# mengyao/Complete-Striped-Smith-Waterman-Library

Hardware: AMD Instinct MI355X
Metric: GCUPS (higher is better)
Workload: dtype int16x2 in a column frame (value + phi(column); 32-bit adds on the packed pair, three-input maxima on the bit patterns); reference u8/int16 semantics; 1 GPU; BASELINE config 2: 100k x 150 bp reads vs 1 Mb target; 2/-2/3/1, score_size 2, flag 0; reads_per_gpu=100000, read_len=150, ref_len=1000000

## Files before the change

complete-striped-smith-waterman-library_amd/csrc/lanes.h:

```cpp
#ifndef SSW_LANES_H
#define SSW_LANES_H

#include <stdint.h>

typedef uint32_t u32;
typedef short s16x2 __attribute__((ext_vector_type(2)));
typedef unsigned short u16x2 __attribute__((ext_vector_type(2)));
typedef uint32_t u32x4 __attribute__((ext_vector_type(4)));
typedef uint32_t u32x2 __attribute__((ext_vector_type(2)));

#ifdef SSW_SIMT_EMU
#include "simt_emu.h"
#else
#include <hip/hip_runtime.h>
#define SSW_DEV __device__ __forceinline__
#define SSW_DEVM __device__ __forceinline__
#define SSW_HD __host__ __device__ inline
#define SSW_DYN_LDS(name) extern __shared__ __attribute__((aligned(16))) unsigned char name[]

SSW_DEV u32 xl_row_shr1_zero(u32 v) { return (u32)__builtin_amdgcn_mov_dpp((int)v, 0x111, 0xf, 0xf, true); }
SSW_DEV u32 xl_row_shr1_keep(u32 keep, u32 v) { return (u32)__builtin_amdgcn_update_dpp((int)keep, (int)v, 0x111, 0xf, 0xf, false); }
SSW_DEV u32 xl_row_shr1_umax(u32 v, u32 b)
{
	u32 r;
// ... 159 lines not shown
{
	const int l = emu::cur->lane, i = l & 15;
	int src = i;
	if (CTRL < 0x100) src = (i & ~3) | ((CTRL >> (2 * (i & 3))) & 3);
	else if ((CTRL & 0x1f0) == 0x100) src = i + (CTRL & 15);
	else if ((CTRL & 0x1f0) == 0x110) src = i - (CTRL & 15);
	else src = (i - (CTRL & 15)) & 15;
	const bool ok = src >= 0 && src < 16 && ((BANK >> (i >> 2)) & 1);
	return emu::exchange(v, (l & ~15) | (src & 15), ok, old);
}
#else
template <int CTRL, int BANK> SSW_DEV u32 xl_dpp_banks(u32 old, u32 v) { return (u32)__builtin_amdgcn_update_dpp((int)old, (int)v, CTRL, 0xf, BANK, false); }
#endif
#define DPP_QUAD_SWAP1 0xB1
#define DPP_QUAD_SWAP2 0x4E

#endif
```

complete-striped-smith-waterman-library_amd/csrc/ssw_host.c:

```c
#include <stdlib.h>
#include <stdio.h>
#include <string.h>
#include <pthread.h>
#include "ssw.h"
#include "ssw_gpu.h"
#ifdef SSW_GPU_TEST_HOOKS
#include "ssw_gpu_diag.h"
#endif
#include "ssw_dev.h"

_Static_assert(sizeof(struct ssw_out_rec) == sizeof(ssw_gpu_result), "device record layout must equal ssw_gpu_result");
_Static_assert(sizeof(struct ssw_best_rec) == sizeof(ssw_gpu_best) && sizeof(ssw_gpu_best) == 16, "device record layout must equal ssw_gpu_best");

struct _profile {
	const int8_t* read;
	const int8_t* mat;
	int32_t readLen;
	int32_t n;
	int8_t score_size;
};

typedef struct { void* p; size_t cap; } dbuf;

typedef struct {
// ... 10 lines not shown
	int overlap;
	int no_track;
	int no_seg_reduce;
	int window_int16;
	int trace_wave;
	int trace_no_lds;
	int trace_waves;
	int trace_unblocked;
	int trace_many;
	int trace_early;
	int trace_w1max, trace_w4max, trace_headroom;
	int pipe_any_count;
	int pipe_low_prio;
	int pipe_parts;
	int no_fill_half;
	int no_pipe;
	int no_lit_spec;
	int trace_no_cls80;
	int trace_diag;
	int serial_buckets;
	int no_dbx;
	int no_tail;
	int no_band;
	int call_trace;
	int db_tsub, dbx_slab;
} ssw_knobs;

#define SSW_TSTREAMS 6
#define SSW_PSTREAMS 7
#define DB_STREAMS 4
// ... 40 lines not shown
#define CALL_TRACE(what) do { if (c->kn.call_trace) fprintf(stderr, "[ssw_gpu call] %9.3f ms  %s\n", dbg_ms(), what); } while (0)

#ifdef SSW_GPU_TEST_HOOKS
static int env_int(const char* name, int dflt) { const char* e = getenv(name); return e && e[0] ? atoi(e) : dflt; }
#endif
static int env_is(const char* name, char ch) { const char* e = getenv(name); return e && e[0] == ch; }
static void knobs_load(ssw_knobs* k)
{
	memset(k, 0, sizeof *k);
	k->debug = getenv("SSW_GPU_DEBUG") != 0;
	k->call_trace = env_is("SSW_GPU_CALL_TRACE", '1');
	k->db_chain_best = 1;
	k->trace_wave = -1;
	k->trace_many = 4096;
	k->trace_w1max = 96; k->trace_w4max = 256; k->trace_headroom = 8;
#ifdef SSW_GPU_TEST_HOOKS
	{ const int v = env_int("SSW_GPU_FRAME_K", 0); k->frame_k = v >= 16 ? v : 0; }
	k->queue_mode = env_is("SSW_GPU_QUEUE", 'j') ? 1 : env_is("SSW_GPU_QUEUE", 's') ? 2 : 0;
	{ const int v = env_int("SSW_GPU_QUEUE_WAVES", 0); k->queue_waves = v > 0 ? v : 0; }
	k->db_plain = env_is("SSW_GPU_DB_FORM", '0');
	k->db_chain_best = !env_is("SSW_GPU_DB_CHAIN_BEST", '0');
	k->xlanes16 = env_int("SSW_GPU_XLANES", 0) == 16;
	{ const int v = env_int("SSW_GPU_XR", 0); k->xr = v >= 1 && v <= 16 ? v : 0; }
	{ const int v = env_int("SSW_GPU_XR_WINDOW", 0); k->xr_window = v >= 1 && v <= 16 ? v : 0; }
	k->fill_plain = env_is("SSW_GPU_FILL_FORM", '0') || env_is("SSW_GPU_FILL_F16", '0');
	k->no_db = env_is("SSW_GPU_NO_DB", '1');
	k->overlap = env_is("SSW_GPU_OVERLAP", '1');
	k->no_track = env_is("SSW_GPU_NO_TRACK", '1');
	k->no_seg_reduce = env_is("SSW_GPU_SEG_REDUCE", '0');
	k->window_int16 = getenv("SSW_GPU_WINDOW_INT16") != 0;
	k->trace_wave = getenv("SSW_GPU_TRACE_WAVE") ? env_is("SSW_GPU_TRACE_WAVE", '1') : -1;
	k->trace_no_lds = env_is("SSW_GPU_TRACE_LDS", '0');
	{ const int v = env_int("SSW_GPU_TRACE_WAVES", 0); k->trace_waves = v == 1 || v == 4 || v == 16 ? v : 0; }
	k->trace_unblocked = env_is("SSW_GPU_TRACE_BLOCKED", '0');
	k->trace_diag = env_is("SSW_GPU_TRACE_DIAG", '1');
	if (getenv("SSW_GPU_TRACE_MANY")) k->trace_many = env_int("SSW_GPU_TRACE_MANY", 4096);
	k->serial_buckets = env_is("SSW_GPU_SERIAL_BUCKETS", '1');
	k->no_dbx = env_is("SSW_GPU_NO_DBX", '1');
	k->no_band = env_is("SSW_GPU_NO_BAND", '1');
	k->trace_no_cls80 = env_is("SSW_GPU_TRACE_CLS80", '0');
	k->no_lit_spec = env_is("SSW_GPU_LIT_SPEC", '0');
	k->no_pipe = env_is("SSW_GPU_PIPE", '0');
	k->no_fill_half = env_is("SSW_GPU_FILL_HALF", '0');
	k->pipe_low_prio = env_is("SSW_GPU_PIPE_PRIO", 'l');
	k->pipe_any_count = env_is("SSW_GPU_PIPE_EVEN", '0');
	{ const int v = env_int("SSW_GPU_TRACE_W1MAX", 0); if (v >= 2 && v <= 254) k->trace_w1max = v; }
	{ const int v = env_int("SSW_GPU_TRACE_W4MAX", 0); if (v >= 2 && v <= 3070) k->trace_w4max = v; }
	{ const int v = env_int("SSW_GPU_TRACE_HEADROOM", 0); if (v >= 2 && v <= 64) k->trace_headroom = v; }
	{ const int v = env_int("SSW_GPU_PIPE_PARTS", 0); k->pipe_parts = v >= 2 && v <= 8 ? v : 0; }
	k->trace_early = env_int("SSW_GPU_TRACE_EARLY", 0);
	k->no_tail = env_is("SSW_GPU_NO_TAIL", '1');
	{ const int v = env_int("SSW_GPU_DB_TSUB", 0); k->db_tsub = v > 0 ? v : 0; }
	{ const int v = env_int("SSW_GPU_DBX_SLAB", 0); k->dbx_slab = v > 0 ? v : 0; }
#endif
}
#ifdef SSW_GPU_TEST_HOOKS
int ssw_gpu_has_test_hooks(void) { return 1; }
// ... 451 lines not shown
	if (key <= SSW_RMAX) { b->R = key; b->strips = 1; b->P16 = 16 * key; b->lanes = 16; b->use_x = 0; return; }
	b->P16 = P16; b->lanes = g->xlanes; b->use_x = 1;
	b->strips = (P16 + g->rows - 1) / g->rows;
	b->R = (P16 + b->lanes * b->strips - 1) / (b->lanes * b->strips);
	if (b->lanes == 64 && b->strips > 1 && g->xrmax > 4 && !g->no_tail) {
		const int32_t rem = P16 - (b->strips - 1) * 64 * g->xrmax, need = (rem + 63) / 64, tr = need <= 1 ? 1 : need <= 2 ? 2 : need <= 4 ? 4 : 0;
		if (rem > 0 && tr > 0 && g->xrmax * (b->strips - 1) + tr < b->R * b->strips) { b->R = g->xrmax; b->tailR = tr; }
	}
}

typedef struct {
	int active, dbl, seg;
	int pipe;
	int32_t tile, halo, ntiles;
	int64_t maxcols, chunk;
	size_t cm_bytes, sg_bytes, bnd_bytes, cand_bytes, q_ints, cs_ints;
	size_t cm_off, sg_off, bnd_off, cand_off, q_off, cs_off;
} bplan;
typedef struct { int32_t key, sub, q; } keyed;
typedef struct { int32_t key, need, q; } tpend;
static int tpend_cmp(const void* a, const void* b)
{
	const tpend* x = (const tpend*)a; const tpend* y = (const tpend*)b;
	if (x->key != y->key) return x->key < y->key ? -1 : 1;
	return x->q < y->q ? -1 : x->q > y->q;
}
static int keyed_cmp(const void* a, const void* b)
{
	const keyed* x = (const keyed*)a; const keyed* y = (const keyed*)b;
	if (x->key != y->key) return x->key < y->key ? -1 : 1;
// ... 1205 lines not shown
	ssw_shim_event_record(e1, c->stream);
	c->tm.fill_launches++;
	for (int32_t q = 0; q < nq; ++q) c->tm.fill_cells += (Q->h_off[q + 1] - Q->h_off[q]) * (int64_t)refLen;
	note_fill_kernel(c, c->tm.fill_cells, &bc->best_fill_cells, "k_literal (lane model of the SSE2 kernels)", 0.0, 0, 1);
	return 0;
}

static void plan_bucket(const ssw_gpu_ctx* c, const batch_call* bc, const target_plan* tp, const bucket* B, bplan* P)
{
	const int32_t refLen = tp->refLen;
	const int64_t stride = tp->stride;
	const int32_t Pq = B->P16, halo_full = halo_for(Pq, bc->maxmat, bc->prm->gapE);
	const int use_x = B->use_x;
	const int gran = use_x ? 1 : 16;
	int32_t tile, halo, ntiles;
	int64_t want = 1;
	int small_call = 0;
	if ((int64_t)halo_full * 8 * gran < refLen) {
		int64_t launch_pairs = use_x ? B->npairs : (int64_t)(c->cm_budget / (size_t)(8 * stride));
		if (launch_pairs < 1) launch_pairs = 1;
		if (launch_pairs > B->npairs) launch_pairs = B->npairs;
		want = (4 * 32768 + B->npairs - 1) / B->npairs;
		if (!use_x && launch_pairs * ((want + 15) / 16) < 6000) want = 16 * ((6000 + launch_pairs - 1) / launch_pairs);
		int64_t maxt = refLen / ((int64_t)halo_full * 8);
		if (want > maxt) want = maxt;
		want = (want + gran - 1) / gran * gran; if (want < gran) want = gran;
	}
	{
		int64_t slots = use_x ? (int64_t)c->dev_wave_slots : (int64_t)c->dev_cus * (c->device_share > 1 ? 96 : 32);
		if (c->device_share > 1) { slots /= c->device_share; if (slots < 256) slots = 256; }
// ... 13 lines not shown
		ntiles = (refLen + tile - 1) / tile; halo = (halo_full + 15) / 16 * 16;
		if (ntiles <= 1) { ntiles = 1; tile = (refLen + 15) / 16 * 16; halo = 0; }
	}
	const int64_t maxcols = (((int64_t)tile + halo < refLen ? (int64_t)tile + halo : refLen) + 31) / 16 * 16;
	int64_t per_pair = 8 * stride + (use_x ? 16 * maxcols * ntiles : 0);
	int64_t chunk = (int64_t)(c->cm_budget / (size_t)per_pair);
	const int dbl = !use_x && chunk < B->npairs && c->kn.overlap;
	const int pipe = !use_x && !dbl && chunk < B->npairs && !c->kn.no_pipe;
	int parts = dbl || pipe ? 2 : 1;
	if (pipe && c->kn.pipe_parts) parts = c->kn.pipe_parts;
	if (parts > 1) chunk = (int64_t)((c->cm_budget / (size_t)parts) / (size_t)per_pair);
	if (chunk < 1) chunk = 1;
	if (chunk > B->npairs) chunk = B->npairs;
	if (!use_x && chunk < B->npairs) {
		const int64_t bpp = (ntiles + 15) / 16;
		int64_t nl = (B->npairs + chunk - 1) / chunk;
		if (pipe && parts > 1 && !c->kn.pipe_any_count && nl % parts) nl += parts - nl % parts;
		int64_t even = (B->npairs + nl - 1) / nl;
		const int64_t ncu = c->dev_cus;
		const int64_t unit = (ncu / (bpp > ncu ? ncu : bpp) > 0 ? ncu / (bpp > ncu ? ncu : bpp) : 1) * (B->half ? 2 : 1);
		even = (even + unit - 1) / unit * unit;
		if (even <= chunk) chunk = even;
		else if (chunk >= unit) chunk = chunk / unit * unit;
		if (B->half && (chunk & 1) && chunk > 1) --chunk;
	}
	memset(P, 0, sizeof *P);
	P->active = 1;
	P->tile = tile; P->halo = halo; P->ntiles = ntiles; P->maxcols = maxcols; P->chunk = chunk; P->dbl = dbl; P->pipe = pipe && chunk < B->npairs ? parts : 0;
	P->seg = !dbl && !c->kn.no_seg_reduce ;
	P->cm_bytes = ALIGN16(4 * stride * chunk) * (P->pipe ? P->pipe : 1);
	P->sg_bytes = P->seg ? ALIGN16(4 * tp->seg_stride * chunk) * (P->pipe ? P->pipe : 1) : 0;
	P->bnd_bytes = use_x ? ALIGN16(16 * maxcols * ntiles * chunk) : 0;
	P->cand_bytes = use_x ? ALIGN16(32 * ntiles * chunk) : 0;
	if (use_x && B->lanes == 64) { P->q_ints = chainq_queue_ints(chunk * ntiles * B->strips); P->cs_ints = chainq_cands_ints(chunk * ntiles * B->strips); }
}

static void plan_target(const ssw_gpu_ctx* c, const batch_call* bc, target_plan* tp, int allow_conc)
{
	tp->max_chunk = 1; tp->nact = 0;
	tp->tot_cm = tp->tot_sg = tp->tot_bnd = tp->tot_cand = tp->tot_q = tp->tot_cs = 0;
	tp->max_cm = tp->max_sg = tp->max_bnd = tp->max_cand = 0;
// ... 86 lines not shown
	if (!half || B->use_x || fa->form != 3 || !ssw_frame_params(&c->kn, top, prm->gapO, prm->gapE, bc->minmat, 8, &hb, &hk)) return 0;
	fa->fr_base = hb; fa->fr_kmask = hk;
	return 1;
}

static void reduce_args_for(const ssw_gpu_ctx* c, const batch_call* bc, const target_plan* tp, const bucket* B, const bplan* P, int32_t p0, int32_t np,
                            const fill_bufs* fb, ssw_reduce_args* ra)
{
	const ssw_gpu_params* prm = bc->prm;
	ra->cm16 = fb->cm16; ra->cm8 = fb->cm8; ra->cm_stride = tp->stride; ra->refLen = tp->refLen; ra->pairs = bc->d_pairs + B->first_pair + p0; ra->npairs = np;
	ra->qoff = bc->Q->d_off; ra->maskLen = prm->maskLen; ra->bias = bc->bias; ra->score_size = prm->score_size;
	ra->flag = prm->flag; ra->filters = prm->filters; ra->res = bc->d_res; ra->cand = bucket_cand(c, tp, B, P); ra->tile = P->tile; ra->ntiles = P->ntiles;
	ra->sg16 = fb->sg16; ra->sg8 = fb->sg8; ra->seg_stride = tp->seg_stride;
}

static int fill_launch(ssw_gpu_ctx* c, batch_call* bc, const target_plan* tp, int b, int32_t p0, int32_t np, const fill_bufs* fb, void* st, int* ndefer)
{
	const bucket* B = &bc->bk[b]; const bplan* P = &tp->bp[b];
	const ssw_gpu_params* prm = bc->prm;
	const int use_x = B->use_x, conc = ndefer != 0;
	const int32_t n = bc->n, refLen = tp->refLen, tile = P->tile, halo = P->halo, ntiles = P->ntiles;
	ssw_fill_args fa;
	const int use_half = fill_args_for(c, bc, tp, B, P, p0, np, fb, B->half && !conc, &fa);
	int xform = 0;
	if (use_x) {
		int32_t xfr_base = 0, xfr_kmask = 0;
		if (bc->fill_form != 0 && B->lanes == 64 &&
		    ssw_frame_params(&c->kn, (int64_t)B->P16 * (bc->maxmat > 0 ? bc->maxmat : 0), prm->gapO, prm->gapE, bc->minmat, 64, &xfr_base, &xfr_kmask)) xform = 3;
		ssw_chainx_args xa; memset(&xa, 0, sizeof xa);
		xa.tgt = tp->d_tgt; xa.refLen = refLen; xa.qcodes = bc->Q->d_codes; xa.qoff = bc->Q->d_off; xa.mat = bc->d_mat; xa.n = n;
		xa.gapO2 = bc->gapO2; xa.gapE2 = bc->gapE2; xa.gapE = prm->gapE; xa.maxmat = bc->maxmat; xa.njobs = np * ntiles;
		xa.pairs = fa.pairs; xa.tile = tile; xa.halo = halo; xa.ntiles = ntiles; xa.cm16 = fb->cm16; xa.cm8 = fb->cm8;
		xa.cm_stride = tp->stride; xa.bnd = (uint32_t*)(tp->base_bnd + P->bnd_off); xa.bnd_stride = P->maxcols; xa.cand = bucket_cand(c, tp, B, P); xa.lanes = B->lanes;
// ... 40 lines not shown
	const int dbl = P->dbl;
	const int pipe = P->pipe;
	const fill_bufs A = bucket_bufs(tp, P);
	fill_bufs B2 = A;
	if (dbl) { B2.cm16 = (uint32_t*)tp->base_cmB16; B2.cm8 = (uint32_t*)tp->base_cmB8; }
	void *pe0 = 0, *pe1 = 0;
	if (pipe) {
		pe0 = next_event(c); pe1 = next_event(c);
		if (ssw_shim_event_record(pe0, c->stream)) return fail(c, "stream wait failed: %s", ssw_shim_last_error());
		for (int k = 0; k < pipe - 1; ++k) {
			if (!c->pstream[k]) { c->pstream[k] = c->kn.pipe_low_prio ? ssw_shim_stream_create_low() : ssw_shim_stream_create(); c->ev_pipe[k] = ssw_shim_event_create(); }
			if (!c->pstream[k] || !c->ev_pipe[k]) return fail(c, "stream creation failed: %s", ssw_shim_last_error());
			if (ssw_shim_stream_wait_event(c->pstream[k], pe0)) return fail(c, "stream wait failed: %s", ssw_shim_last_error());
		}
	}
	int launch_i = 0;
	for (int32_t p0 = 0; p0 < B->npairs; p0 += (int32_t)P->chunk, ++launch_i) {
		const int32_t np = B->npairs - p0 < P->chunk ? B->npairs - p0 : (int32_t)P->chunk;
		const int bi = pipe ? launch_i % pipe : dbl ? (launch_i & 1) : 0;
		void* st = c->stream;
		fill_bufs fb = bi ? B2 : A;
		if (pipe) {
			if (bi) st = c->pstream[bi - 1];
			fb.cm16 = (uint32_t*)((unsigned char*)A.cm16 + (size_t)bi * (P->cm_bytes / (size_t)pipe)); fb.cm8 = (uint32_t*)((unsigned char*)A.cm8 + (size_t)bi * (P->cm_bytes / (size_t)pipe));
			fb.sg16 = P->seg ? (uint32_t*)((unsigned char*)A.sg16 + (size_t)bi * (P->sg_bytes / (size_t)pipe)) : 0;
			fb.sg8 = P->seg ? (uint32_t*)((unsigned char*)A.sg8 + (size_t)bi * (P->sg_bytes / (size_t)pipe)) : 0;
		}
		if (dbl && launch_i >= 2) ssw_shim_stream_wait_event(c->stream, c->ev_red[bi]);
		void *e0 = 0, *e1 = 0;
		if (!pipe) { e0 = next_event(c); e1 = next_event(c); ssw_shim_event_record(e0, st); }
		if (fill_launch(c, bc, tp, b, p0, np, &fb, st, 0)) return -1;
		if (!pipe) ssw_shim_event_record(e1, st);
		c->tm.fill_launches++; if (pipe) c->tm.fill_pipelined++;
		ssw_reduce_args ra;
		reduce_args_for(c, bc, tp, B, P, p0, np, &fb, &ra);
		if (dbl) {
			ssw_shim_event_record(c->ev_fill[bi], c->stream);
			ssw_shim_stream_wait_event(c->stream2, c->ev_fill[bi]);
			if (ssw_shim_launch_reduce(&ra, c->stream2)) return fail(c, "reduce launch failed: %s", ssw_shim_last_error());
			ssw_shim_event_record(c->ev_red[bi], c->stream2);
		} else
		if (ssw_shim_launch_reduce(&ra, st)) return fail(c, "reduce launch failed: %s", ssw_shim_last_error());
	}
	if (dbl) {
		ssw_shim_stream_wait_event(c->stream, c->ev_red[0]);
		if (launch_i > 1) ssw_shim_stream_wait_event(c->stream, c->ev_red[1]);
// ... 89 lines not shown
	if (ssw_shim_event_record(ge0, c->stream) || ssw_shim_event_record(c->ev_db, c->stream)) return fail(c, "event record failed: %s", ssw_shim_last_error());
	for (int i = 0; i < nb; ++i) border[i] = i;
	for (int i = 1; i < nb; ++i) {
		const int v = border[i]; int j = i;
		while (j > 0 && (int64_t)bk[border[j - 1]].npairs * bk[border[j - 1]].P16 < (int64_t)bk[v].npairs * bk[v].P16) { border[j] = border[j - 1]; --j; }
		border[j] = v;
	}
	const int strip_sx = 5;
	if (side_stream_join_in(c, strip_sx, side_used)) return -1;
	for (int pass_x = 0; pass_x < 2; ++pass_x) {
		for (int bi_ = 0; bi_ < nb; ++bi_) {
			const int b = border[bi_];
			const bucket* B = &bk[b]; const bplan* P = &tp->bp[b];
			if (!P->active || (B->use_x != 0) != pass_x) continue;
			const fill_bufs fb = bucket_bufs(tp, P);
			if (fill_launch(c, bc, tp, b, 0, B->npairs, &fb, c->tstream[strip_sx], &ndefer)) return -1;
			reduce_args_for(c, bc, tp, B, P, 0, B->npairs, &fb, &bc->rdefer[nrdefer++]);
		}
		if (pass_x == 0 && ndefer > 0 && fill_deferred_grids(c, bc, ndefer, side_used)) return -1;
	}
	if (side_streams_join_out(c, side_used)) return -1;
	if (nrdefer > 0 && reduce_deferred_grid(c, bc->rdefer, nrdefer)) return -1;
	ssw_shim_event_record(ge1, c->stream);
	c->tm.fill_launches++;
	return 0;
}

static int window_phase(ssw_gpu_ctx* c, const batch_call* bc, const target_plan* tp)
{
	const bucket* bk = bc->bk; const int nb = bc->nb; const int32_t n = bc->n;
	win_in wi; memset(&wi, 0, sizeof wi);
// ... 1417 lines not shown
```

complete-striped-smith-waterman-library_amd/csrc/ssw_kernels.hip:

```cpp
#include "lanes.h"
#include "ssw_dev.h"

#define DEAD2 0x80008000u

SSW_DEV int vm_query(const ssw_vmap& m, int v) { return m.vq ? m.vq[v] : v; }
SSW_DEV const int8_t* vm_target(const ssw_vmap& m, const int8_t* tgt, int v) { return m.vq ? m.tcodes + (m.win ? m.win[m.vt[v]].start : m.toff[m.vt[v]]) : tgt; }

#define RING_BYTES 160
#define CHAIN_BYTES (RING_BYTES + 256 + 256)

template <int R> struct ChainGeom {
	static constexpr int C = (R + 3) / 4;
	static constexpr int PSTRIDE = C * 256;
	static constexpr int A8 = 16 * R - 8;
	static constexpr int TAP = A8 / R;
	static constexpr int K8 = A8 % R;
};

template <int R, int PM = 0>
SSW_DEV void build_profile(unsigned char* lds, u32 base, int first, int nthreads,
                           const int8_t* mat, int n,
                           const int8_t* qa, int lena, int reva,
                           const int8_t* qb, int lenb, int p16a = 0x7fffffff, int p16b = 0x7fffffff, int gapE = 0)
{
// ... 233 lines not shown
	for (int base = nsteps - 32; base < nsteps; base += 16)
		if (base >= 0) fill_flush16<R, FORM>(lds, out16, out8, base, l16, store_from, ncols, o16, o8, g16, g8, a.fr_base, a.fr_kmask, gapEi);
}

template <int R, int FORM>
__global__ void __launch_bounds__(256) SSW_WAVES_PER_EU(R <= 10 ? 7 : 1, 8) k_fill(ssw_fill_args a)
{
	SSW_DYN_LDS(lds);
	fill_body<R, FORM>(a, (int)blockIdx.x, lds);
}

#define CRING8_BYTES 128
#define VRING8_BYTES 288
#define PARK8_BYTES 192
#define CHAIN8_BYTES (RING_BYTES + 2 * CRING8_BYTES + 2 * VRING8_BYTES + 2 * PARK8_BYTES + 16)

template <int R> struct Rows8 { u32 v; Rows8<R - 1> up; };
template <> struct Rows8<1> { u32 v; };
template <int I, int R> SSW_DEV u32& row_at(Rows8<R>& a) { if constexpr (I == 0) return a.v; else return row_at<I - 1>(a.up); }
template <int... I> struct RowSeq {};
template <int N, int... I> struct RowSeqTo : RowSeqTo<N - 1, N - 1, I...> {};
template <int... I> struct RowSeqTo<0, I...> { typedef RowSeq<I...> type; };
template <int R, int... I> SSW_DEV void rows_set(Rows8<R>& a, u32 v, RowSeq<I...>) { ((row_at<I>(a) = v), ...); }
template <int R, int... I> SSW_DEV void rows_sub(Rows8<R>& a, u32 k, RowSeq<I...>) { ((row_at<I>(a) -= k), ...); }

template <int R, int r>
SSW_DEV void chain_row8(const u32x4* sc, Rows8<R>& H, Rows8<R>& E, u32& x, u32& f, u32& cm, u32 c1, u32 gapE2, u32 fl)
{
	u32& Hr = row_at<r>(H); u32& Er = row_at<r>(E);
	const u32 xn = r + 1 < R ? Hr + sc[(r + 1) >> 2][(r + 1) & 3] : 0u;
// ... 25 lines not shown
		const int c = rem >> 6, l = (rem & 63) >> 2, k = rem & 3;
		const int ch = l >> 3, r = c * 4 + k, row = (l & 7) * R + r;
		u32 v;
		if (b == n || (ch && !live1)) v = fr_pack(FR_DEAD, FR_DEAD);
		else if (r >= R) v = 0;
		else {
			int lo = 0, hi = 0;
			if (row < len[2 * ch]) lo = mat[b * n + q[2 * ch][row]];
			if (q[2 * ch + 1] && row < len[2 * ch + 1]) hi = mat[b * n + q[2 * ch + 1][row]];
			v = fr_pack(lo + gapE, hi + gapE);
		}
		lds_st32(lds, (u32)w * 4u, v);
	}
}

SSW_DEV void fill_stage8(unsigned char* lds, u32 rbl, int s1, bool low8, u32 lgd, int fr_base, int fr_kmask, int gapE, u32 gE2)
{
	const u32 ph = pk_dup(fr_base + ((s1 & fr_kmask) + 2) * gapE) + lgd;
	const u32 sc = rbl + 2 * PARK8_BYTES + 4u * ((u32)s1 & 16u), sv = rbl + 2 * PARK8_BYTES + 2 * CRING8_BYTES + 4u * ((u32)s1 & 48u);
	const bool mir = ((u32)s1 & 48u) == 0 && low8;
#pragma unroll
	for (u32 ch = 0; ch < 2; ++ch) {
		const u32 p = rbl + ch * PARK8_BYTES;
		const u32 cm = lds_ld32(lds, p), f = lds_ld32(lds, p + 64u), h = lds_ld32(lds, p + 128u);
		const u32 vv = pk_max3_fr(f, h + 2u * gE2, ph) - ph;
		lds_st32(lds, sc + ch * CRING8_BYTES, cm - (ph - gE2));
		lds_st32(lds, sv + ch * VRING8_BYTES, vv);
		if (mir) lds_st32(lds, sv + ch * VRING8_BYTES + 256u, vv);
	}
}

SSW_DEV void fill_flush8(unsigned char* lds, u32 rb, int base, int l16, int store_from, int ncols, bool live1,
                         uint32_t* o16, uint32_t* o8, int64_t cm_stride, uint32_t* gq, int gapE, int gapO)
{
	const int tc = base + l16;
	const bool in = tc >= store_from && tc < ncols;
	const u32 ca = rb + 2 * PARK8_BYTES + 4u * ((u32)(tc + 7) & 31u), va = rb + 2 * PARK8_BYTES + 2 * CRING8_BYTES + 4u * ((u32)(tc - 1) & 63u);
	const u32 carry = rb + 2 * PARK8_BYTES + 2 * CRING8_BYTES + 2 * VRING8_BYTES;
	const int lg = l16 * gapE;
	const u32 up = pk_dup(lg), dn = pk_dup(-lg - gapO);
	u32 i16[2], i8[2];
#pragma unroll
	for (u32 ch = 0; ch < 2; ++ch) {
		i8[ch] = lds_ld32(lds, ca + ch * CRING8_BYTES);
		u32 v[9];
#pragma unroll
		for (int k = 0; k < 9; ++k) v[k] = lds_ld32(lds, va + ch * VRING8_BYTES + 4u * k);
		u32 w = pk_max3_nonneg(v[1], v[2], v[3]);
		w = pk_max3_nonneg(w, v[4], v[5]);
		w = pk_max3_nonneg(w, v[6], v[7]);
		w = pk_max3_nonneg(w, v[8], i8[ch]);
		u32 x = v[0] + up;
		const u32 y = l16 == 15 ? lds_ld32(lds, carry + 4u * ch) : x;
		x = pk_max(x, xl_row_ror<1>(y));
		x = pk_max(x, xl_row_shr_zero<2>(x));
		x = pk_max(x, xl_row_shr_zero<4>(x));
		x = pk_max(x, xl_row_shr_zero<8>(x));
		if (l16 == 15) lds_st32(lds, carry + 4u * ch, pk_adds(x, pk_dup(-16 * gapE)));
		i16[ch] = pk_max(w, pk_adds(x, dn));
	}
	if (in) {
		o16[tc] = i16[0]; o8[tc] = i8[0];
		if (live1) { o16[cm_stride + tc] = i16[1]; o8[cm_stride + tc] = i8[1]; }
	}
	if (gq) {
		u32 m[4];
#pragma unroll
		for (int k = 0; k < 4; ++k) m[k] = in ? (k & 1 ? i8[k >> 1] : i16[k >> 1]) : 0u;
		const u32 x16 = pk_max(xl_dpp_banks<0x128, 0xc>(m[0], m[2]), xl_dpp_banks<0x128, 0x3>(m[2], m[0]));
		const u32 x8 = pk_max(xl_dpp_banks<0x128, 0xc>(m[1], m[3]), xl_dpp_banks<0x128, 0x3>(m[3], m[1]));
		u32 y = pk_max(xl_dpp_banks<0x114, 0xa>(x16, x8), xl_dpp_banks<0x104, 0x5>(x8, x16));
		y = pk_max(y, xl_dpp_banks<DPP_QUAD_SWAP1, 0xf>(y, y));
		y = pk_max(y, xl_dpp_banks<DPP_QUAD_SWAP2, 0xf>(y, y));
		if ((l16 & 3) == 0 && (live1 || l16 < 8) && base >= store_from && base < ncols) gq[base >> 4] = y;
	}
}

template <int R>
SSW_DEV void fill_body8(const ssw_fill_args& a, const int bid, unsigned char* lds)
{
	typedef ChainGeom<R> G;
	constexpr int C = G::C;
	const int tid = (int)threadIdx.x, l16 = tid & 15, grp = tid >> 4, ch = l16 & 1, pos = l16 >> 1;
	const int pg = bid / a.bpp, tchunk = bid - pg * a.bpp;
	const bool live1 = 2 * pg + 1 < a.npairs;
	const int gapEi = (int)(a.gapE2 & 0xffffu), gapOi = (int)(a.gapO2 & 0xffffu);
	const u32 prof_bytes = (u32)(a.n + 1) * G::PSTRIDE;
	const u32 ring = prof_bytes + (u32)grp * CHAIN8_BYTES;
	const u32 rb = opaque(ring + RING_BYTES), outv = rb + 2 * PARK8_BYTES + 2 * CRING8_BYTES, carry = outv + 2 * VRING8_BYTES;
	const u32 nulloff = (u32)a.n * G::PSTRIDE;

	{
		const int8_t* q[4]; int len[4];
#pragma unroll
		for (int k = 0; k < 2; ++k) {
			const ssw_pair pr = a.pairs[k && !live1 ? 2 * pg : 2 * pg + k];
			q[2 * k] = a.qcodes + a.qoff[pr.qa];
			len[2 * k] = (int)(a.qoff[pr.qa + 1] - a.qoff[pr.qa]);
			q[2 * k + 1] = pr.qb >= 0 ? a.qcodes + a.qoff[pr.qb] : (const int8_t*)0;
			len[2 * k + 1] = pr.qb >= 0 ? (int)(a.qoff[pr.qb + 1] - a.qoff[pr.qb]) : 0;
		}
		build_profile8<R>(lds, tid, 256, a.mat, a.n, q, len, live1, gapEi);
	}

	const int t = tchunk * 16 + grp;
	const bool active = t < a.ntiles;
	const int tile_lo = active ? t * a.tile : 0;
	const int tile_hi = active ? (tile_lo + a.tile < a.refLen ? tile_lo + a.tile : a.refLen) : 0;
	const int c_first = tile_lo - a.halo > 0 ? tile_lo - a.halo : 0;
	const int ncols = tile_hi - c_first;
	int maxcols = a.tile + a.halo; if (maxcols > a.refLen) maxcols = a.refLen;
	const int nsteps = (maxcols + 8 + 15) & ~15;
	const int8_t* tg = a.tgt + c_first;
	uint32_t* o16 = a.cm16 + (int64_t)(2 * pg) * a.cm_stride + c_first;
	uint32_t* o8 = a.cm8 + (int64_t)(2 * pg) * a.cm_stride + c_first;
	const int store_from = tile_lo - c_first;
	uint32_t* gq = a.sg16 ? (l16 & 4 ? a.sg8 : a.sg16) + (int64_t)(2 * pg + (l16 >> 3)) * a.seg_stride + (c_first >> 4) : (uint32_t*)0;

	lds_st16(lds, ring + 2u * (48 + l16), nulloff);
	{
		int code = l16 < ncols ? tg[l16] : a.n;
		if (code < 0 || code > a.n) code = a.n;
		const u32 off = (u32)code * G::PSTRIDE;
		lds_st16(lds, ring + 2u * l16, off);
		lds_st16(lds, ring + 2u * (64 + l16), off);
	}
#pragma unroll
	for (int k = 0; k < 9; ++k) lds_st32(lds, outv + 4u * (u32)(l16 + 16 * k), 0u);
	if (l16 < 2) lds_st32(lds, carry + 4u * l16, 0u);
	u32 nxt;
	{
		const int tc = 16 + l16;
		int code = tc < ncols ? tg[tc] : a.n;
		if (code < 0 || code > a.n) code = a.n;
		nxt = (u32)code * G::PSTRIDE;
	}
	__syncthreads();

	const u32 zero0 = pk_dup(fr_phi(0, pos, 8, a.fr_base, a.fr_kmask, gapEi) - gapEi);
	u32 fl = zero0 + a.gapE2;
	typedef typename RowSeqTo<R>::type Rows;
	Rows8<R> H, E;
	rows_set(H, zero0, Rows()); rows_set(E, fl, Rows());
	u32 Hlast = zero0, Fout = zero0 + a.gapE2, cmout = zero0, hsave = zero0;
	const u32 lane_prof = (u32)(ch * 8 + pos) * 16u;
	const u32 gO = a.gapO2 - a.gapE2, gE = a.gapE2;
	const u32 gEv = opaque(gE);
	u32 fin = 0;
	const u32 park = rb + (u32)ch * PARK8_BYTES, rbl = opaque(rb + 4u * (u32)l16);
	const u32 lgd = pk_dup(l16 * gapEi);
	const bool low8 = l16 < 8;

	for (int s0 = 0; s0 < nsteps; s0 += 16) {
		if (s0 > 0 && (s0 & a.fr_kmask) == 0) {
			const u32 k = (u32)(a.fr_kmask + 1) * a.gapE2;
			rows_sub(H, k, Rows()); rows_sub(E, k, Rows());
			Hlast -= k; Fout -= k; cmout -= k; hsave -= k; fl -= k;
		}
		{
			const int p = (s0 + 16 + l16) & 63;
			lds_st16(lds, ring + 2u * p, nxt);
			if (p < 16) lds_st16(lds, ring + 2u * (64 + p), nxt);
			const int tc = s0 + 32 + l16;
			int code = tc < ncols ? tg[tc] : a.n;
			if (code < 0 || code > a.n) code = a.n;
			nxt = (u32)code * G::PSTRIDE;
		}
		wave_lds_fence();
		if (s0 >= 16) fill_stage8(lds, rbl, s0 - 16, low8, lgd, a.fr_base, a.fr_kmask, gapEi, gE);
		wave_lds_fence();
		if (s0 >= 32)
			fill_flush8(lds, rb, s0 - 32, l16, store_from, ncols, live1, o16, o8, a.cm_stride, gq, gapEi, gapOi);
		const u32 rp = ring + 2u * (u32)((s0 - pos) & 63);
#pragma unroll
		for (int j = 0; j < 16; ++j) {
			const u32 paddr = lds_ld16(lds, rp + 2u * j) + lane_prof;
			u32x4 sc[C];
#pragma unroll
			for (int c = 0; c < C; ++c) sc[c] = lds_ld128(lds, paddr + 256u * c);
			const u32 hprev = Hlast;
			const u32 hin = xl_row_shr2_umax(Hlast, fl); fl += gE;
			xl_row_shr2_sub_keep(fin, Fout, gEv);
			u32 f = fin, d = hsave;
			u32 cm = xl_row_shr2_zero(cmout);
			chain_rows_fr8(sc, H, E, d, f, cm, gO, gE, fl, Rows());
			hsave = hin; Hlast = row_at<R - 1>(H); Fout = f; cmout = cm;
			if (pos == 7) {
				lds_st32(lds, park + 4u * j, cm); lds_st32(lds, park + 64u + 4u * j, f); lds_st32(lds, park + 128u + 4u * j, hprev);
			}
		}
	}
	wave_lds_fence();
	fill_stage8(lds, rbl, nsteps - 16, low8, lgd, a.fr_base, a.fr_kmask, gapEi, gE);
	wave_lds_fence();
	for (int base = nsteps - 32; base < nsteps; base += 16)
		if (base >= 0) fill_flush8(lds, rb, base, l16, store_from, ncols, live1, o16, o8, a.cm_stride, gq, gapEi, gapOi);
}

template <int R>
__global__ void __launch_bounds__(256) SSW_WAVES_PER_EU(R <= 9 ? 7 : R <= 15 ? 5 : 4, 8) k_fill8(ssw_fill_args a)
{
	SSW_DYN_LDS(lds);
	fill_body8<R>(a, (int)blockIdx.x, lds);
}

template <int CLS> struct FillClass { static constexpr int LO = CLS == 0 ? 1 : CLS == 1 ? 11 : 17, HI = CLS == 0 ? 10 : CLS == 1 ? 16 : 24; };
template <int R, int CLS, int FORM> SSW_DEV void fillm_case(const ssw_fill_args& a, int bid, unsigned char* lds)
{
	if (R >= FillClass<CLS>::LO && R <= FillClass<CLS>::HI) fill_body<(R >= FillClass<CLS>::LO && R <= FillClass<CLS>::HI) ? R : FillClass<CLS>::LO, FORM>(a, bid, lds);
}
template <int CLS, int FORM>
// ... 3843 lines not shown
```

Before: 11070 GCUPS.

## Add narrower-tile tail launches to pipelined fill and streamline fill8 ring addressing

The host planner now switches the last launches of a pipelined, half-bucket fill series to smaller pair chunks over more, narrower target tiles. This is meant to shrink the pipeline drain where the final launches leave the GPU underfilled. Separately, the 8-row fill kernel precomputes per-lane LDS ring and output pointers, drops per-column modulo address arithmetic, simplifies target-code clamping, and folds the carry into a three-input max. The tail planning adds new heuristics, and the reworked ring wrap and mirror stores carry a correctness risk.

New measurement: 11150 GCUPS, median of 6. About the same (+0.7%).

```diff
diff --git a/complete-striped-smith-waterman-library_amd/csrc/lanes.h b/complete-striped-smith-waterman-library_amd/csrc/lanes.h
--- a/complete-striped-smith-waterman-library_amd/csrc/lanes.h
+++ b/complete-striped-smith-waterman-library_amd/csrc/lanes.h
@@ -197,5 +197,15 @@
 #endif
 #define DPP_QUAD_SWAP1 0xB1
 #define DPP_QUAD_SWAP2 0x4E
-
-#endif
+#ifdef SSW_SIMT_EMU
+template <int CTRL> SSW_DEV u32 xl_quad_perm(u32 v) { return xl_dpp_banks<CTRL, 0xf>(v, v); }
+#else
+template <int CTRL> SSW_DEV u32 xl_quad_perm(u32 v) { return (u32)__builtin_amdgcn_mov_dpp((int)v, CTRL, 0xf, 0xf, true); }
+#endif
+#ifdef SSW_SIMT_EMU
+SSW_DEV u32 opaque_uniform(u32 v) { return v; }
+#else
+SSW_DEV u32 opaque_uniform(u32 v) { asm("" : "+s"(v)); return v; }
+#endif
+
+#endif
diff --git a/complete-striped-smith-waterman-library_amd/csrc/ssw_host.c b/complete-striped-smith-waterman-library_amd/csrc/ssw_host.c
--- a/complete-striped-smith-waterman-library_amd/csrc/ssw_host.c
+++ b/complete-striped-smith-waterman-library_amd/csrc/ssw_host.c
@@ -48,6 +48,7 @@
 	int pipe_low_prio;
 	int pipe_parts;
 	int no_fill_half;
+	int pipe_tail;
 	int no_pipe;
 	int no_lit_spec;
 	int trace_no_cls80;
@@ -118,6 +119,7 @@
 	k->trace_wave = -1;
 	k->trace_many = 4096;
 	k->trace_w1max = 96; k->trace_w4max = 256; k->trace_headroom = 8;
+	k->pipe_tail = 1;
 #ifdef SSW_GPU_TEST_HOOKS
 	{ const int v = env_int("SSW_GPU_FRAME_K", 0); k->frame_k = v >= 16 ? v : 0; }
 	k->queue_mode = env_is("SSW_GPU_QUEUE", 'j') ? 1 : env_is("SSW_GPU_QUEUE", 's') ? 2 : 0;
@@ -145,6 +147,7 @@
 	k->trace_no_cls80 = env_is("SSW_GPU_TRACE_CLS80", '0');
 	k->no_lit_spec = env_is("SSW_GPU_LIT_SPEC", '0');
 	k->no_pipe = env_is("SSW_GPU_PIPE", '0');
+	k->pipe_tail = env_is("SSW_GPU_PIPE_TAIL", '0') ? 0 : env_is("SSW_GPU_PIPE_TAIL", 'f') ? 2 : 1;
 	k->no_fill_half = env_is("SSW_GPU_FILL_HALF", '0');
 	k->pipe_low_prio = env_is("SSW_GPU_PIPE_PRIO", 'l');
 	k->pipe_any_count = env_is("SSW_GPU_PIPE_EVEN", '0');
@@ -626,6 +629,8 @@
 	int pipe;
 	int32_t tile, halo, ntiles;
 	int64_t maxcols, chunk;
+	int32_t tail_tile, tail_ntiles, tail_from;
+	int64_t tail_chunk;
 	size_t cm_bytes, sg_bytes, bnd_bytes, cand_bytes, q_ints, cs_ints;
 	size_t cm_off, sg_off, bnd_off, cand_off, q_off, cs_off;
 } bplan;
@@ -1861,6 +1866,8 @@
 	const int use_x = B->use_x;
 	const int gran = use_x ? 1 : 16;
 	int32_t tile, halo, ntiles;
+	int32_t tail_tile = 0, tail_ntiles = 0, tail_from = 0;
+	int64_t tail_chunk = 0;
 	int64_t want = 1;
 	int small_call = 0;
 	if ((int64_t)halo_full * 8 * gran < refLen) {
@@ -1904,6 +1911,7 @@
 	if (chunk > B->npairs) chunk = B->npairs;
 	if (!use_x && chunk < B->npairs) {
 		const int64_t bpp = (ntiles + 15) / 16;
+		const int64_t cmax = chunk;
 		int64_t nl = (B->npairs + chunk - 1) / chunk;
 		if (pipe && parts > 1 && !c->kn.pipe_any_count && nl % parts) nl += parts - nl % parts;
 		int64_t even = (B->npairs + nl - 1) / nl;
@@ -1913,8 +1921,33 @@
 		if (even <= chunk) chunk = even;
 		else if (chunk >= unit) chunk = chunk / unit * unit;
 		if (B->half && (chunk & 1) && chunk > 1) --chunk;
+		const int64_t nreg = (B->npairs + chunk - 1) / chunk - parts;
+		if (pipe && parts > 1 && B->half && c->kn.pipe_tail && nreg >= parts && (!small_call || c->kn.pipe_tail == 2)) {
+			const int force = c->kn.pipe_tail == 2;
+			int64_t tw = (int64_t)ntiles * 4;
+			const int64_t maxt = refLen / ((int64_t)halo_full * 8) / gran * gran;
+			if (!force && tw > maxt) tw = maxt;
+			const int32_t tt = tw > 0 ? (int32_t)(((refLen + tw - 1) / tw + 15) / 16 * 16) : tile;
+			const int32_t tn = (refLen + tt - 1) / tt;
+			const int64_t hold = ncu * (B->half <= 9 ? 6 : B->half <= 15 ? 5 : 4), tbpp = (tn + 15) / 16;
+			const int64_t tunit = (hold / tbpp > 0 ? hold / tbpp : 1) * 2;
+			int64_t rest = B->npairs - nreg * cmax;
+			int64_t tc = rest > 0 ? (rest + parts - 1) / parts : 0;
+			if (force) { if (tc < 2) tc = 2; }
+			else { if (tc < 2 * tunit) tc = 2 * tunit; tc = (tc + tunit - 1) / tunit * tunit; }
+			tc &= ~(int64_t)1;
+			if (tn >= 2 * ntiles && tt >= 16 && tc >= 2 && (force ? tc <= cmax : 2 * tc <= cmax) && parts * tc < B->npairs) {
+				int64_t big = (B->npairs - parts * tc + nreg - 1) / nreg;
+				if (!force && big >= unit) big = (big + unit - 1) / unit * unit;
+				if (big > cmax) big = cmax;
+				if (big & 1) ++big;
+				if (big > cmax) big -= 2;
+				if (big >= tc && big >= 2) { chunk = big; tail_tile = tt; tail_ntiles = tn; tail_chunk = tc; tail_from = (int32_t)nreg; }
+			}
+		}
 	}
 	memset(P, 0, sizeof *P);
+	P->tail_tile = tail_tile; P->tail_ntiles = tail_ntiles; P->tail_chunk = tail_chunk; P->tail_from = tail_from;
 	P->active = 1;
 	P->tile = tile; P->halo = halo; P->ntiles = ntiles; P->maxcols = maxcols; P->chunk = chunk; P->dbl = dbl; P->pipe = pipe && chunk < B->npairs ? parts : 0;
 	P->seg = !dbl && !c->kn.no_seg_reduce ;
@@ -2031,9 +2064,9 @@
 	ra->sg16 = fb->sg16; ra->sg8 = fb->sg8; ra->seg_stride = tp->seg_stride;
 }
 
-static int fill_launch(ssw_gpu_ctx* c, batch_call* bc, const target_plan* tp, int b, int32_t p0, int32_t np, const fill_bufs* fb, void* st, int* ndefer)
-{
-	const bucket* B = &bc->bk[b]; const bplan* P = &tp->bp[b];
+static int fill_launch(ssw_gpu_ctx* c, batch_call* bc, const target_plan* tp, int b, int32_t p0, int32_t np, const fill_bufs* fb, void* st, int* ndefer, const bplan* geom)
+{
+	const bucket* B = &bc->bk[b]; const bplan* P = geom ? geom : &tp->bp[b];
 	const ssw_gpu_params* prm = bc->prm;
 	const int use_x = B->use_x, conc = ndefer != 0;
 	const int32_t n = bc->n, refLen = tp->refLen, tile = P->tile, halo = P->halo, ntiles = P->ntiles;
@@ -2104,9 +2137,16 @@
 			if (ssw_shim_stream_wait_event(c->pstream[k], pe0)) return fail(c, "stream wait failed: %s", ssw_shim_last_error());
 		}
 	}
+	bplan tailP = *P;
+	if (P->tail_chunk) { tailP.tile = P->tail_tile; tailP.ntiles = P->tail_ntiles; }
+	if (c->kn.debug) fprintf(stderr, "[ssw_gpu] fill series: %d pairs, %lld per launch in %d tiles of %d (+%d), %d parts; tails from launch %d: %lld pairs in %d tiles of %d\n",
+	                         B->npairs, (long long)P->chunk, P->ntiles, P->tile, P->halo, pipe, P->tail_chunk ? P->tail_from : -1, (long long)P->tail_chunk, P->tail_ntiles, P->tail_tile);
 	int launch_i = 0;
-	for (int32_t p0 = 0; p0 < B->npairs; p0 += (int32_t)P->chunk, ++launch_i) {
-		const int32_t np = B->npairs - p0 < P->chunk ? B->npairs - p0 : (int32_t)P->chunk;
+	int32_t step = 0;
+	for (int32_t p0 = 0; p0 < B->npairs; p0 += step, ++launch_i) {
+		const int tail = P->tail_chunk && launch_i >= P->tail_from;
+		step = (int32_t)(tail ? P->tail_chunk : P->chunk);
+		const int32_t np = B->npairs - p0 < step ? B->npairs - p0 : step;
 		const int bi = pipe ? launch_i % pipe : dbl ? (launch_i & 1) : 0;
 		void* st = c->stream;
 		fill_bufs fb = bi ? B2 : A;
@@ -2119,7 +2159,7 @@
 		if (dbl && launch_i >= 2) ssw_shim_stream_wait_event(c->stream, c->ev_red[bi]);
 		void *e0 = 0, *e1 = 0;
 		if (!pipe) { e0 = next_event(c); e1 = next_event(c); ssw_shim_event_record(e0, st); }
-		if (fill_launch(c, bc, tp, b, p0, np, &fb, st, 0)) return -1;
+		if (fill_launch(c, bc, tp, b, p0, np, &fb, st, 0, tail ? &tailP : 0)) return -1;
 		if (!pipe) ssw_shim_event_record(e1, st);
 		c->tm.fill_launches++; if (pipe) c->tm.fill_pipelined++;
 		ssw_reduce_args ra;
@@ -2239,7 +2279,7 @@
 			const bucket* B = &bk[b]; const bplan* P = &tp->bp[b];
 			if (!P->active || (B->use_x != 0) != pass_x) continue;
 			const fill_bufs fb = bucket_bufs(tp, P);
-			if (fill_launch(c, bc, tp, b, 0, B->npairs, &fb, c->tstream[strip_sx], &ndefer)) return -1;
+			if (fill_launch(c, bc, tp, b, 0, B->npairs, &fb, c->tstream[strip_sx], &ndefer, 0)) return -1;
 			reduce_args_for(c, bc, tp, B, P, 0, B->npairs, &fb, &bc->rdefer[nrdefer++]);
 		}
 		if (pass_x == 0 && ndefer > 0 && fill_deferred_grids(c, bc, ndefer, side_used)) return -1;
diff --git a/complete-striped-smith-waterman-library_amd/csrc/ssw_kernels.hip b/complete-striped-smith-waterman-library_amd/csrc/ssw_kernels.hip
--- a/complete-striped-smith-waterman-library_amd/csrc/ssw_kernels.hip
+++ b/complete-striped-smith-waterman-library_amd/csrc/ssw_kernels.hip
@@ -271,6 +271,9 @@
 #define VRING8_BYTES 288
 #define PARK8_BYTES 192
 #define CHAIN8_BYTES (RING_BYTES + 2 * CRING8_BYTES + 2 * VRING8_BYTES + 2 * PARK8_BYTES + 16)
+#define CM8_OFF (2u * PARK8_BYTES)
+#define V8_OFF (CM8_OFF + 2u * CRING8_BYTES)
+#define CARRY8_OFF (V8_OFF + 2u * VRING8_BYTES)
 
 template <int R> struct Rows8 { u32 v; Rows8<R - 1> up; };
 template <> struct Rows8<1> { u32 v; };
@@ -326,54 +329,56 @@
 	}
 }
 
-SSW_DEV void fill_stage8(unsigned char* lds, u32 rbl, int s1, bool low8, u32 lgd, int fr_base, int fr_kmask, int gapE, u32 gE2)
-{
-	const u32 ph = pk_dup(fr_base + ((s1 & fr_kmask) + 2) * gapE) + lgd;
-	const u32 sc = rbl + 2 * PARK8_BYTES + 4u * ((u32)s1 & 16u), sv = rbl + 2 * PARK8_BYTES + 2 * CRING8_BYTES + 4u * ((u32)s1 & 48u);
-	const bool mir = ((u32)s1 & 48u) == 0 && low8;
+SSW_DEV void fill_stage8(unsigned char* lds, u32 rbl, int s1, bool low7, bool last, u32 lgd, int fr_base, int fr_kmask, int gapE, u32 gE2)
+{
+	const u32 ph = opaque_uniform(pk_dup(fr_base + ((s1 & fr_kmask) + 2) * gapE)) + lgd;
+	const u32 t16 = (u32)s1 & 16u, t48 = (u32)s1 & 48u;
+	const u32 sc = rbl + 4u * t16, sv = rbl + 4u * t48;
+	const bool wrapc = t16 == 0 && low7, mir = t48 == 0 && low7, wrapv = t48 == 48 && last;
 #pragma unroll
 	for (u32 ch = 0; ch < 2; ++ch) {
 		const u32 p = rbl + ch * PARK8_BYTES;
 		const u32 cm = lds_ld32(lds, p), f = lds_ld32(lds, p + 64u), h = lds_ld32(lds, p + 128u);
 		const u32 vv = pk_max3_fr(f, h + 2u * gE2, ph) - ph;
-		lds_st32(lds, sc + ch * CRING8_BYTES, cm - (ph - gE2));
-		lds_st32(lds, sv + ch * VRING8_BYTES, vv);
-		if (mir) lds_st32(lds, sv + ch * VRING8_BYTES + 256u, vv);
-	}
-}
-
-SSW_DEV void fill_flush8(unsigned char* lds, u32 rb, int base, int l16, int store_from, int ncols, bool live1,
-                         uint32_t* o16, uint32_t* o8, int64_t cm_stride, uint32_t* gq, int gapE, int gapO)
-{
-	const int tc = base + l16;
-	const bool in = tc >= store_from && tc < ncols;
-	const u32 ca = rb + 2 * PARK8_BYTES + 4u * ((u32)(tc + 7) & 31u), va = rb + 2 * PARK8_BYTES + 2 * CRING8_BYTES + 4u * ((u32)(tc - 1) & 63u);
-	const u32 carry = rb + 2 * PARK8_BYTES + 2 * CRING8_BYTES + 2 * VRING8_BYTES;
+		const u32 cv = cm - (ph - gE2);
+		if (wrapc) { lds_st32(lds, sc + CM8_OFF + 100u + ch * CRING8_BYTES, cv); sched_fence(); }
+		else lds_st32(lds, sc + CM8_OFF - 28u + ch * CRING8_BYTES, cv);
+		lds_st32(lds, sv + V8_OFF + 4u + ch * VRING8_BYTES, vv);
+		if (mir) lds_st32(lds, sv + V8_OFF + 260u + ch * VRING8_BYTES, vv);
+		if (wrapv) lds_st32(lds, sv + V8_OFF - 252u + ch * VRING8_BYTES, vv);
+	}
+}
+
+SSW_DEV void fill_flush8(unsigned char* lds, u32 rb, u32 rbl, int base, int l16, int in_lo, int in_hi, int ncols, bool live1,
+                         uint32_t* o16l, uint32_t* o8l, int64_t cm_stride, uint32_t* gq, int gapE, int gapO)
+{
+	const bool from = base >= in_lo, in = from && base < in_hi;
+	const u32 ca = rbl + 4u * ((u32)base & 16u), va = rbl + 4u * ((u32)base & 48u);
+	const u32 carry = rb + CARRY8_OFF;
 	const int lg = l16 * gapE;
 	const u32 up = pk_dup(lg), dn = pk_dup(-lg - gapO);
 	u32 i16[2], i8[2];
 #pragma unroll
 	for (u32 ch = 0; ch < 2; ++ch) {
-		i8[ch] = lds_ld32(lds, ca + ch * CRING8_BYTES);
+		i8[ch] = lds_ld32(lds, ca + CM8_OFF + ch * CRING8_BYTES);
 		u32 v[9];
 #pragma unroll
-		for (int k = 0; k < 9; ++k) v[k] = lds_ld32(lds, va + ch * VRING8_BYTES + 4u * k);
+		for (int k = 0; k < 9; ++k) v[k] = lds_ld32(lds, va + V8_OFF + ch * VRING8_BYTES + 4u * k);
 		u32 w = pk_max3_nonneg(v[1], v[2], v[3]);
 		w = pk_max3_nonneg(w, v[4], v[5]);
 		w = pk_max3_nonneg(w, v[6], v[7]);
 		w = pk_max3_nonneg(w, v[8], i8[ch]);
 		u32 x = v[0] + up;
-		const u32 y = l16 == 15 ? lds_ld32(lds, carry + 4u * ch) : x;
-		x = pk_max(x, xl_row_ror<1>(y));
+		x = pk_max3_nonneg(x, xl_row_shr_zero<1>(x), lds_ld32(lds, carry + 4u * ch));
 		x = pk_max(x, xl_row_shr_zero<2>(x));
 		x = pk_max(x, xl_row_shr_zero<4>(x));
 		x = pk_max(x, xl_row_shr_zero<8>(x));
-		if (l16 == 15) lds_st32(lds, carry + 4u * ch, pk_adds(x, pk_dup(-16 * gapE)));
+		if (l16 == 15) lds_st32(lds, carry + 4u * ch, pk_subu(x, pk_dup(16 * gapE)));
 		i16[ch] = pk_max(w, pk_adds(x, dn));
 	}
 	if (in) {
-		o16[tc] = i16[0]; o8[tc] = i8[0];
-		if (live1) { o16[cm_stride + tc] = i16[1]; o8[cm_stride + tc] = i8[1]; }
+		o16l[base] = i16[0]; o8l[base] = i8[0];
+		if (live1) { o16l[cm_stride + base] = i16[1]; o8l[cm_stride + base] = i8[1]; }
 	}
 	if (gq) {
 		u32 m[4];
@@ -382,11 +387,13 @@
 		const u32 x16 = pk_max(xl_dpp_banks<0x128, 0xc>(m[0], m[2]), xl_dpp_banks<0x128, 0x3>(m[2], m[0]));
 		const u32 x8 = pk_max(xl_dpp_banks<0x128, 0xc>(m[1], m[3]), xl_dpp_banks<0x128, 0x3>(m[3], m[1]));
 		u32 y = pk_max(xl_dpp_banks<0x114, 0xa>(x16, x8), xl_dpp_banks<0x104, 0x5>(x8, x16));
-		y = pk_max(y, xl_dpp_banks<DPP_QUAD_SWAP1, 0xf>(y, y));
-		y = pk_max(y, xl_dpp_banks<DPP_QUAD_SWAP2, 0xf>(y, y));
-		if ((l16 & 3) == 0 && (live1 || l16 < 8) && base >= store_from && base < ncols) gq[base >> 4] = y;
-	}
-}
+		y = pk_max(y, xl_quad_perm<DPP_QUAD_SWAP1>(y));
+		y = pk_max(y, xl_quad_perm<DPP_QUAD_SWAP2>(y));
+		if ((l16 & 3) == 0 && (live1 || l16 < 8) && from && base < ncols) gq[base >> 4] = y;
+	}
+}
+
+SSW_DEV int tgt_code8(int code, int n) { return (u32)code < (u32)n ? code : n; }
 
 template <int R>
 SSW_DEV void fill_body8(const ssw_fill_args& a, const int bid, unsigned char* lds)
@@ -399,7 +406,7 @@
 	const int gapEi = (int)(a.gapE2 & 0xffffu), gapOi = (int)(a.gapO2 & 0xffffu);
 	const u32 prof_bytes = (u32)(a.n + 1) * G::PSTRIDE;
 	const u32 ring = prof_bytes + (u32)grp * CHAIN8_BYTES;
-	const u32 rb = opaque(ring + RING_BYTES), outv = rb + 2 * PARK8_BYTES + 2 * CRING8_BYTES, carry = outv + 2 * VRING8_BYTES;
+	const u32 rb = opaque(ring + RING_BYTES), outv = rb + V8_OFF, carry = rb + CARRY8_OFF;
 	const u32 nulloff = (u32)a.n * G::PSTRIDE;
 
 	{
@@ -424,15 +431,15 @@
 	int maxcols = a.tile + a.halo; if (maxcols > a.refLen) maxcols = a.refLen;
 	const int nsteps = (maxcols + 8 + 15) & ~15;
 	const int8_t* tg = a.tgt + c_first;
-	uint32_t* o16 = a.cm16 + (int64_t)(2 * pg) * a.cm_stride + c_first;
-	uint32_t* o8 = a.cm8 + (int64_t)(2 * pg) * a.cm_stride + c_first;
+	uint32_t* o16l = a.cm16 + (int64_t)(2 * pg) * a.cm_stride + c_first + l16;
+	uint32_t* o8l = a.cm8 + (int64_t)(2 * pg) * a.cm_stride + c_first + l16;
 	const int store_from = tile_lo - c_first;
+	const int in_lo = store_from - l16, in_hi = ncols - l16;
 	uint32_t* gq = a.sg16 ? (l16 & 4 ? a.sg8 : a.sg16) + (int64_t)(2 * pg + (l16 >> 3)) * a.seg_stride + (c_first >> 4) : (uint32_t*)0;
 
 	lds_st16(lds, ring + 2u * (48 + l16), nulloff);
 	{
-		int code = l16 < ncols ? tg[l16] : a.n;
-		if (code < 0 || code > a.n) code = a.n;
+		const int code = tgt_code8(l16 < ncols ? tg[l16] : a.n, a.n);
 		const u32 off = (u32)code * G::PSTRIDE;
 		lds_st16(lds, ring + 2u * l16, off);
 		lds_st16(lds, ring + 2u * (64 + l16), off);
@@ -440,13 +447,7 @@
 #pragma unroll
 	for (int k = 0; k < 9; ++k) lds_st32(lds, outv + 4u * (u32)(l16 + 16 * k), 0u);
 	if (l16 < 2) lds_st32(lds, carry + 4u * l16, 0u);
-	u32 nxt;
-	{
-		const int tc = 16 + l16;
-		int code = tc < ncols ? tg[tc] : a.n;
-		if (code < 0 || code > a.n) code = a.n;
-		nxt = (u32)code * G::PSTRIDE;
-	}
+	int nxt = 16 < in_hi ? tg[16 + l16] : a.n;
 	__syncthreads();
 
 	const u32 zero0 = pk_dup(fr_phi(0, pos, 8, a.fr_base, a.fr_kmask, gapEi) - gapEi);
@@ -461,7 +462,9 @@
 	u32 fin = 0;
 	const u32 park = rb + (u32)ch * PARK8_BYTES, rbl = opaque(rb + 4u * (u32)l16);
 	const u32 lgd = pk_dup(l16 * gapEi);
-	const bool low8 = l16 < 8;
+	const bool low7 = l16 < 7, last = l16 == 15;
+	const u32 ringl = opaque(ring + 2u * (u32)l16), ringp = opaque(ring - 2u * (u32)pos);
+	const int8_t* tgl = tg + 32 + l16;
 
 	for (int s0 = 0; s0 < nsteps; s0 += 16) {
 		if (s0 > 0 && (s0 & a.fr_kmask) == 0) {
@@ -470,20 +473,18 @@
 			Hlast -= k; Fout -= k; cmout -= k; hsave -= k; fl -= k;
 		}
 		{
-			const int p = (s0 + 16 + l16) & 63;
-			lds_st16(lds, ring + 2u * p, nxt);
-			if (p < 16) lds_st16(lds, ring + 2u * (64 + p), nxt);
-			const int tc = s0 + 32 + l16;
-			int code = tc < ncols ? tg[tc] : a.n;
-			if (code < 0 || code > a.n) code = a.n;
-			nxt = (u32)code * G::PSTRIDE;
+			const u32 g = (u32)(s0 + 16) & 48u;
+			const u32 off = (u32)tgt_code8(nxt, a.n) * G::PSTRIDE;
+			lds_st16(lds, ringl + 2u * g, off);
+			if (g == 0) lds_st16(lds, ringl + 128u, off);
+			nxt = s0 + 32 < in_hi ? tgl[s0] : a.n;
 		}
 		wave_lds_fence();
-		if (s0 >= 16) fill_stage8(lds, rbl, s0 - 16, low8, lgd, a.fr_base, a.fr_kmask, gapEi, gE);
+		if (s0 >= 16) fill_stage8(lds, rbl, s0 - 16, low7, last, lgd, a.fr_base, a.fr_kmask, gapEi, gE);
 		wave_lds_fence();
 		if (s0 >= 32)
-			fill_flush8(lds, rb, s0 - 32, l16, store_from, ncols, live1, o16, o8, a.cm_stride, gq, gapEi, gapOi);
-		const u32 rp = ring + 2u * (u32)((s0 - pos) & 63);
+			fill_flush8(lds, rb, rbl, s0 - 32, l16, in_lo, in_hi, ncols, live1, o16l, o8l, a.cm_stride, gq, gapEi, gapOi);
+		const u32 rp = ringp + 2u * (((u32)s0 & 48u) == 0 ? 64u : (u32)s0 & 48u);
 #pragma unroll
 		for (int j = 0; j < 16; ++j) {
 			const u32 paddr = lds_ld16(lds, rp + 2u * j) + lane_prof;
@@ -503,10 +504,10 @@
 		}
 	}
 	wave_lds_fence();
-	fill_stage8(lds, rbl, nsteps - 16, low8, lgd, a.fr_base, a.fr_kmask, gapEi, gE);
+	fill_stage8(lds, rbl, nsteps - 16, low7, last, lgd, a.fr_base, a.fr_kmask, gapEi, gE);
 	wave_lds_fence();
 	for (int base = nsteps - 32; base < nsteps; base += 16)
-		if (base >= 0) fill_flush8(lds, rb, base, l16, store_from, ncols, live1, o16, o8, a.cm_stride, gq, gapEi, gapOi);
+		if (base >= 0) fill_flush8(lds, rb, rbl, base, l16, in_lo, in_hi, ncols, live1, o16l, o8l, a.cm_stride, gq, gapEi, gapOi);
 }
 
 template <int R>
```
